# CVLAB-Unibo/MM2D3D

Measured on AMD Instinct MI355X. Metric: LiDAR scenes/sec fwd+bwd (NuScenes ~35k pts, 5cm voxel), higher is better.
Workload: dtype fp16 MFMA, fp32 accumulate, loss scale 65536 on the device (2D branch: IEEE fp16 maps and packed weights - the reference's precision: 16 = fp16 autocast + GradScaler) + f32 (3D sparse branch, fp32 as in the reference: f32 MFMA on narrow layers, fp32-faithful 3-term split-bf16 products with fp32 accu; 1 GPU; BASELINE.json configs[1]: NuScenes-shaped (32x1090 sweep, 34,880 pts/scene), 5 cm voxels, 480x302 RGB + sparse depth; full two-domain training step (train.py:186-292): 2D+3D fwd on source and target, 2 CE + 4 KL, backward, AdamW x2 + OneCycle; distinct_batches_rotated=4, parallelism=dp1

## Files before the change

include/mm2d3d.h:

```cpp
#ifndef MM2D3D_H
#define MM2D3D_H

#include <stddef.h>
#include <stdint.h>

#ifdef __cplusplus
extern "C" {
#endif

typedef void* mm_stream_t;

#define MM_OK 0
#define MM_ERR_ARG (-1)
#define MM_ERR_HIP (-2)
#define MM_ERR_WORKSPACE (-3)
#define MM_ERR_UNSUPPORTED (-4)

const char* mm_last_error(void);

typedef void* mm_handle_t;
size_t mm_handle_sync_bytes(void);
size_t mm_handle_fault_bytes(void);
int mm_create(int device_id, void* sync_dev, size_t sync_bytes, void* fault_host, size_t fault_bytes, mm_handle_t* out);
int mm_destroy(mm_handle_t h);
// ... 7 lines not shown
int mm_fault_poll(mm_handle_t h);


int64_t mm_hash_capacity(int64_t n_items);
size_t mm_dedupe_ws_bytes(int64_t n_bound);

int mm_voxel_dedupe(const void* coords, int coords_is_i64, int64_t n_bound, const int32_t* n_dev, int shift,
                    uint64_t* tkeys, int32_t* tvals, int64_t cap, int32_t* item2vox, int32_t* vox_coords,
                    int32_t* csr_off, int32_t* csr_items, int32_t* n_active_dev, int32_t* err_dev, int no_spin, void* ws,
                    size_t ws_bytes, mm_stream_t stream);

int mm_batch_lower_bound(const int32_t* vox_coords, const int32_t* n_dev, int32_t split, int32_t* out, mm_stream_t stream);
int mm_subm_neighbors(const int32_t* vox_coords, int64_t n, int32_t spatial_size, const uint64_t* tkeys,
                      const int32_t* tvals, int64_t cap, int32_t* nbr, mm_stream_t stream);

int mm_down_neighbors(const int32_t* vox_coords_fine, int64_t n_fine, const int32_t* fine2coarse, int64_t n_coarse,
                      int32_t* nbr, mm_stream_t stream);

size_t mm_rulebook_ws_bytes(int64_t n_out, int K);
int mm_rulebook_compact(const int32_t* nbr, int K, int64_t n_out, int32_t* rin, int32_t* rout, int32_t* offsets,
                        int32_t* csr_off, int32_t* csr_pos, int no_spin, void* ws, size_t ws_bytes, mm_stream_t stream);
int mm_rulebook_csr(const int32_t* nbr, int K, int64_t n_out, int32_t* csr_off, int32_t* csr_pos, int no_spin, void* ws,
                    size_t ws_bytes, mm_stream_t stream);

size_t mm_voxelize_ws_bytes(int64_t n_total, int B);
int mm_voxelize_batch(const float* points, const int32_t* scene_off_dev, const int32_t* scene_off_host, int B, const float* rot,
                      const double* u, int transl, float scale, int full_scale, int64_t* locs, int32_t* keep, int32_t* counts,
                      float* min_value, double* offset, void* ws, size_t ws_bytes, mm_stream_t stream);
size_t mm_voxelize_ws_bytes_f64(int64_t n_total, int B);
int mm_voxelize_batch_f64(const double* points, const int32_t* scene_off_dev, const int32_t* scene_off_host, int B, const float* rot,
                          const double* u, int transl, double scale, int full_scale, int64_t* locs, int32_t* keep, int32_t* counts,
                          double* min_value, double* offset, void* ws, size_t ws_bytes, mm_stream_t stream);
int mm_project_batch(const float* points_img, const float* depth_vals, const int64_t* labels, const int32_t* scene_off_dev,
                     const int32_t* scene_off_host, int B, int H, int W, const uint8_t* flip, int64_t* img_indices, float* depth,
                     double* seg2d, int32_t* winner, int32_t* err, mm_stream_t stream);
int mm_collect_points(const int32_t* keep, const int32_t* n_keep_dev, int64_t n_bound, const int64_t* locs, const int64_t* img_indices,
                      const int64_t* labels, const float* image, int C, int H, int W, const float* points, int64_t* img_indices_out,
                      int64_t* labels_out, float* feats_out, float* points_out, mm_stream_t stream);
int mm_collect_points_f64(const int32_t* keep, const int32_t* n_keep_dev, int64_t n_bound, const int64_t* locs, const int64_t* img_indices,
                          const int64_t* labels, const float* image, int C, int H, int W, const double* points, int64_t* img_indices_out,
                          int64_t* labels_out, float* feats_out, double* points_out, mm_stream_t stream);
int mm_collect_points_dev(const int32_t* keep, const int32_t* counts_dev, int B, int64_t n_total, const int64_t* locs,
                          const int64_t* img_indices, const int64_t* labels, const float* image, int C, int H, int W, const float* points,
                          int64_t* img_indices_out, int64_t* labels_out, float* feats_out, float* points_out,
                          const void* const* extra_in, void* const* extra_out, int n_extra, int extra_bytes, mm_stream_t stream);
int mm_collect_points_f64_dev(const int32_t* keep, const int32_t* counts_dev, int B, int64_t n_total, const int64_t* locs,
// ... 394 lines not shown
```

mm2d3d_amd/_lib.py:

```python
from __future__ import annotations

import contextlib
import ctypes as C
import os
import subprocess

import torch

_HERE = os.path.dirname(os.path.abspath(__file__))
LIB_PATH = os.environ.get("MM_LIB_PATH") or os.path.join(_HERE, "libmm2d3d_hip.so")
CSRC = os.path.join(_HERE, "csrc")

_lib = None

vp, i32, i64, sz, f32, f64 = C.c_void_p, C.c_int32, C.c_int64, C.c_size_t, C.c_float, C.c_double

_PROTOS = {
    "mm_last_error": (C.c_char_p, []),
    "mm_handle_sync_bytes": (sz, []),
    "mm_handle_fault_bytes": (sz, []),
    "mm_create": (i32, [i32, vp, sz, vp, sz, C.POINTER(vp)]),
    "mm_destroy": (i32, [vp]),
    "mm_set_option": (i32, [vp, i32, i32]),
    "mm_get_option": (i32, [vp, i32]),
    "mm_fault_poll": (i32, [vp]),
    "mm_hash_capacity": (i64, [i64]),
    "mm_dedupe_ws_bytes": (sz, [i64]),
    "mm_voxel_dedupe": (i32, [vp, i32, i64, vp, i32, vp, vp, i64, vp, vp, vp, vp, vp, vp, i32, vp, sz, vp]),
    "mm_batch_lower_bound": (i32, [vp, vp, i32, vp, vp]),
    "mm_subm_neighbors": (i32, [vp, i64, i32, vp, vp, i64, vp, vp]),
    "mm_down_neighbors": (i32, [vp, i64, vp, i64, vp, vp]),
    "mm_rulebook_ws_bytes": (sz, [i64, i32]),
    "mm_rulebook_compact": (i32, [vp, i32, i64, vp, vp, vp, vp, vp, i32, vp, sz, vp]),
    "mm_rulebook_csr": (i32, [vp, i32, i64, vp, vp, i32, vp, sz, vp]),
    "mm_spconv_ws_bytes": (sz, [i64, i32, i32, i32]),
    "mm_spconv_apply": (i32, [vp, i32, i32, vp, i32, i32, i64, vp, vp, vp, vp, i32, vp, vp, i32, vp, i64, i32, i32, i32, i32, vp, sz, vp]),
    "mm_spconv_apply_packed": (i32, [vp, i32, i32, vp, i32, i32, i64, vp, vp, vp, vp, i32, vp, vp, i32, vp, i64, i32, i32, i32, vp, i32, vp, sz, vp]),
    "mm_spconv_dw_ws_bytes": (sz, [vp, i32, i32, i32]),
    "mm_spconv_dw": (i32, [vp, i32, i32, vp, i32, i32, vp, vp, vp, i32, vp, i32, i32, vp, sz, vp]),
    "mm_voxelize_ws_bytes": (sz, [i64, i32]),
    "mm_voxelize_batch": (i32, [vp, vp, vp, i32, vp, vp, i32, f32, i32, vp, vp, vp, vp, vp, vp, sz, vp]),
    "mm_project_batch": (i32, [vp, vp, vp, vp, vp, i32, i32, i32, vp, vp, vp, vp, vp, vp, vp]),
    "mm_voxelize_ws_bytes_f64": (sz, [i64, i32]),
    "mm_voxelize_batch_f64": (i32, [vp, vp, vp, i32, vp, vp, i32, f64, i32, vp, vp, vp, vp, vp, vp, sz, vp]),
    "mm_collect_points": (i32, [vp, vp, i64, vp, vp, vp, vp, i32, i32, i32, vp, vp, vp, vp, vp, vp]),
    "mm_collect_points_f64": (i32, [vp, vp, i64, vp, vp, vp, vp, i32, i32, i32, vp, vp, vp, vp, vp, vp]),
    "mm_collect_points_dev": (i32, [vp, vp, i32, i64, vp, vp, vp, vp, i32, i32, i32, vp, vp, vp, vp, vp, vp, vp, i32, i32, vp]),
    "mm_collect_points_f64_dev": (i32, [vp, vp, i32, i64, vp, vp, vp, vp, i32, i32, i32, vp, vp, vp, vp, vp, vp, vp, i32, i32, vp]),
    "mm_image_prepare": (i32, [vp, i64, vp, vp, i32, i32, i32, vp, i64, vp, vp, vp, i64, vp, vp, vp, vp]),
    "mm_jpeg_ws_bytes": (sz, [i32, i64, i64, i64, i64, i64]),
    "mm_jpeg_decode": (i32, [vp, i64, vp, vp, i32, vp, i64, vp, i64, vp, i64, vp, vp, sz, vp]),
    "mm_up_neighbors": (i32, [vp, i64, vp, vp, vp]),
    "mm_os_table_ws_bytes": (sz, [i64, i32]),
    "mm_os_table_build": (i32, [vp, i32, i64, i32, i32, vp, vp, vp, vp, sz, vp]),
    "mm_spconv_os_pack_bytes": (sz, [i32, i32, i32]),
    "mm_spconv_os_pack_blocks": (i64, [i32, i32, i32]),
    "mm_spconv_os_pack_desc_fields": (i32, []),
# ... 118 lines not shown
    "mm_copy_rows_bf16": (i32, [vp, i64, vp, i64, i64, i32, vp]),
    "mm_concat_bf16": (i32, [vp, vp, i32, vp, i64, i32, vp]),
    "mm_maxpool3x3s2_fwd": (i32, [vp, i32, i32, i32, i32, i32, vp, vp, vp]),
    "mm_maxpool3x3s2_bwd": (i32, [vp, i32, vp, i32, vp, i32, i32, i32, i32, vp, vp]),
    "mm_head_ws_bytes": (sz, [i32, i32, i32, i32, i32, i32, i32]),
    "mm_head_fwd": (i32, [vp, i32, i32, i32, i32, i32, i32, i32, vp, vp, i32, vp, vp, sz, vp]),
    "mm_head_bwd": (i32, [vp, i32, i32, i32, i32, i32, i32, i32, vp, i32, vp, vp, vp, vp, sz, vp]),
}


class Bn2dFwdArgs(C.Structure):
    _fields_ = [("x", C.c_void_p), ("ld_x", C.c_int), ("res", C.c_void_p), ("ld_r", C.c_int), ("weight", C.c_void_p), ("bias", C.c_void_p),
                ("running_mean", C.c_void_p), ("running_var", C.c_void_p), ("num_batches_tracked", C.c_void_p), ("y", C.c_void_p),
                ("ld_y", C.c_int), ("save_mean", C.c_void_p), ("save_invstd", C.c_void_p)]


class Bn2dBwdArgs(C.Structure):
    _fields_ = [("x", C.c_void_p), ("ld_x", C.c_int), ("dy", C.c_void_p), ("ld_dy", C.c_int), ("dy2", C.c_void_p), ("ld_dy2", C.c_int),
                ("yout", C.c_void_p), ("ld_y", C.c_int), ("weight", C.c_void_p), ("bias", C.c_void_p), ("save_mean", C.c_void_p),
                ("save_invstd", C.c_void_p), ("dx", C.c_void_p), ("ld_dx", C.c_int), ("dres", C.c_void_p), ("ld_dr", C.c_int),
                ("dweight", C.c_void_p), ("dbias", C.c_void_p)]


class HipLibraryMissing(RuntimeError):
    pass


H16_2D = {
    "mm_conv2d_gemm": "mm_conv2d_gemm_f16",
    "mm_conv2d_dgrad_s2": "mm_conv2d_dgrad_s2_f16",
    "mm_conv2d_3x3s1": "mm_conv2d_3x3s1_f16",
    "mm_conv2d_3x3s1_pair": "mm_conv2d_3x3s1_pair_f16",
    "mm_conv2d_gemm_stat_rows": "mm_conv2d_gemm_stat_rows_f16",
    "mm_conv2d_3x3s1_stat_rows": "mm_conv2d_3x3s1_stat_rows_f16",
    "mm_bn2d_fwd_train_pre": "mm_bn2d_fwd_train_pre_f16",
    "mm_bn2d_single_launch": "mm_bn2d_single_launch_f16",
    "mm_bn2d_fwd_train_pair": "mm_bn2d_fwd_train_pair_f16",
    "mm_bn2d_fwd_train_pre_pool": "mm_bn2d_fwd_train_pre_pool_f16",
    "mm_bn2d_bwd_pool": "mm_bn2d_bwd_pool_f16",
    "mm_bn2d_bwd_pair": "mm_bn2d_bwd_pair_f16",
    "mm_conv2d_wgrad_ws_bytes": "mm_conv2d_wgrad_ws_bytes_f16",
    "mm_conv2d_wgrad": "mm_conv2d_wgrad_f16",
    "mm_conv2d_wgrad3x3_pair": "mm_conv2d_wgrad3x3_pair_f16",
    "mm_conv2d_wgrad_slabs": "mm_conv2d_wgrad_slabs_f16",
    "mm_conv2d_wgrad3x3_pair_slabs": "mm_conv2d_wgrad3x3_pair_slabs_f16",
    "mm_conv2d_wgrad_reduce_desc_bytes": "mm_conv2d_wgrad_reduce_desc_bytes_f16",
# ... 225 lines not shown
```

mm2d3d_amd/csrc/meta.hip:

```cpp
#include "common.h"

namespace {

constexpr unsigned long long EMPTY_KEY = 0xFFFFFFFFFFFFFFFFull;
constexpr int T = 256;

__device__ inline unsigned long long pack_key(int x, int y, int z, int b) {
  return ((unsigned long long)(unsigned)b << 48) | ((unsigned long long)(unsigned)x << 32) |
         ((unsigned long long)(unsigned)y << 16) | (unsigned long long)(unsigned)z;
}

__device__ inline unsigned long long mix64(unsigned long long k) {
  k ^= k >> 33;
  k *= 0xff51afd7ed558ccdull;
  k ^= k >> 33;
  k *= 0xc4ceb9fe1a85ec53ull;
  k ^= k >> 33;
  return k;
}

__device__ inline int hash_find(const unsigned long long* __restrict__ tkeys, const int32_t* __restrict__ tvals,
                                long long mask, unsigned long long key) {
  long long slot = (long long)(mix64(key) & (unsigned long long)mask);
  for (long long probe = 0; probe <= mask; probe++) {
// ... 186 lines not shown
  int64_t o = (int64_t)blockIdx.x * T + threadIdx.x;
  if (o >= n_out) return;
  int e = csr_off[o];
  for (int k = 0; k < K; k++)
    if (nbr[(int64_t)k * n_out + o] >= 0) csr_pos[e++] = pos[(int64_t)k * n_out + o];
}

__global__ void k_fill_i32(int32_t* p, int64_t n, int32_t v) {
  int64_t i = (int64_t)blockIdx.x * blockDim.x + threadIdx.x;
  if (i < n) p[i] = v;
}

inline unsigned nblk(int64_t n) { return (unsigned)mm_cdiv(n > 0 ? n : 1, T); }

__global__ void k_batch_lower_bound(const int32_t* __restrict__ coords, const int32_t* __restrict__ n_dev, int32_t split,
                                    int32_t* __restrict__ out) {
  int lo = 0, hi = *n_dev;
  while (lo < hi) {
    int mid = (lo + hi) >> 1;
    if (coords[(int64_t)mid * 4 + 3] < split) lo = mid + 1;
    else hi = mid;
  }
  *out = lo;
}
}

extern "C" {

int64_t mm_hash_capacity(int64_t n_items) {
  int64_t c = 1024;
  while (c < 2 * n_items) c <<= 1;
  return c;
}

size_t mm_dedupe_ws_bytes(int64_t n) { return 4 * mm_align((size_t)(n + 1) * 4) + mm_scan_ws_bytes(n + 1) + 1024; }

int mm_voxel_dedupe(const void* coords, int coords_is_i64, int64_t n_bound, const int32_t* n_dev, int shift,
                    uint64_t* tkeys, int32_t* tvals, int64_t cap, int32_t* item2vox, int32_t* vox_coords,
                    int32_t* csr_off, int32_t* csr_items, int32_t* n_active_dev, int32_t* err_dev, int no_spin, void* ws,
                    size_t ws_bytes, hipStream_t s) {
  MM_CHECK_ARG(n_bound >= 0 && cap >= 2 * n_bound && (cap & (cap - 1)) == 0, "dedupe: cap must be pow2 >= 2n (n=%lld cap=%lld)",
               (long long)n_bound, (long long)cap);
  MM_CHECK_ARG(shift >= 0 && shift < 16, "dedupe: bad shift %d", shift);
  MMArena ar(ws, ws_bytes);
  int32_t* slot_of = ar.take<int32_t>(n_bound + 1);
  int32_t* flag = ar.take<int32_t>(n_bound + 1);
// ... 82 lines not shown
  if (!pos || !cnt || !scan_ws) {
    mm_set_error("rulebook_compact: workspace too small (%zu < %zu)", ws_bytes, mm_rulebook_ws_bytes(n_out, K));
    return MM_ERR_WORKSPACE;
  }
  int rc = mm_exclusive_scan_nonneg_i32(nbr, pos, total, scan_ws, sws, s, no_spin);
  if (rc) return rc;
  if (rin) hipLaunchKernelGGL(k_emit_rules, dim3(nblk(n_out), K), dim3(T), 0, s, nbr, pos, n_out, K, rin, rout, offsets, pos + total);
  if (csr_off) {
    hipLaunchKernelGGL(k_row_counts, dim3(nblk(n_out)), dim3(T), 0, s, nbr, n_out, K, cnt);
    rc = mm_exclusive_scan_i32(cnt, csr_off, n_out, csr_off + n_out, scan_ws, sws, s, no_spin);
    if (rc) return rc;
    hipLaunchKernelGGL(k_row_fill, dim3(nblk(n_out)), dim3(T), 0, s, nbr, pos, n_out, K, csr_off, csr_pos);
  }
  MM_LAUNCH_CHECK();
  return MM_OK;
}

int mm_rulebook_csr(const int32_t* nbr, int K, int64_t n_out, int32_t* csr_off, int32_t* csr_pos, int no_spin, void* ws, size_t ws_bytes,
                    hipStream_t s) {
  MM_CHECK_ARG(csr_off && csr_pos, "rulebook_csr: null output");
  return mm_rulebook_compact(nbr, K, n_out, nullptr, nullptr, nullptr, csr_off, csr_pos, no_spin, ws, ws_bytes, s);
}

int mm_batch_lower_bound(const int32_t* vox_coords, const int32_t* n_dev, int32_t split, int32_t* out, hipStream_t s) {
  MM_CHECK_ARG(vox_coords && n_dev && out, "batch_lower_bound: null pointer");
  hipLaunchKernelGGL(k_batch_lower_bound, dim3(1), dim3(1), 0, s, vox_coords, n_dev, split, out);
  MM_LAUNCH_CHECK();
  return MM_OK;
}

}
```

mm2d3d_amd/csrc/scan.hip:

```cpp
#include <stdarg.h>

#include <rocprim/device/device_scan.hpp>
#include <rocprim/iterator/counting_iterator.hpp>
#include <rocprim/iterator/transform_iterator.hpp>

#include "common.h"

static thread_local char g_err[512] = "";
void mm_set_error(const char* fmt, ...) {
  va_list ap;
  va_start(ap, fmt);
  vsnprintf(g_err, sizeof(g_err), fmt, ap);
  va_end(ap);
}
extern "C" const char* mm_last_error() { return g_err; }

namespace {
constexpr int SCAN_T = 256;
constexpr int SCAN_PER = 8;
constexpr int SCAN_BLK = SCAN_T * SCAN_PER;

__device__ inline int wave_incl_scan(int v) {
  const int lane = threadIdx.x & 63;
#pragma unroll
// ... 15 lines not shown
  for (int i = 0; i < SCAN_T / 64; i++) {
    int x = wsum[i];
    if (i < w) base += x;
    total += x;
  }
  __syncthreads();
  *tot = total;
  return base + inc - v;
}

template <bool FLAG>
__global__ __launch_bounds__(SCAN_T) void k_block_sums(const int32_t* __restrict__ in, int32_t* __restrict__ sums,
                                                        int64_t n) {
  int64_t base = (int64_t)blockIdx.x * SCAN_BLK + threadIdx.x * SCAN_PER;
  int v = 0;
#pragma unroll
  for (int i = 0; i < SCAN_PER; i++)
    if (base + i < n) v += FLAG ? (in[base + i] >= 0 ? 1 : 0) : in[base + i];
  int tot;
  block_excl_scan(v, &tot);
  if (threadIdx.x == 0) sums[blockIdx.x] = tot;
}

__global__ __launch_bounds__(SCAN_T) void k_scan_sums(int32_t* __restrict__ sums, int64_t nb,
                                                       int32_t* __restrict__ total_out) {
  int carry = 0;
  for (int64_t b0 = 0; b0 < nb; b0 += SCAN_T) {
    int64_t i = b0 + threadIdx.x;
    int v = i < nb ? sums[i] : 0;
    int tot;
    int ex = block_excl_scan(v, &tot);
    if (i < nb) sums[i] = carry + ex;
    carry += tot;
  }
  if (threadIdx.x == 0 && total_out) *total_out = carry;
}

template <bool FLAG>
__global__ __launch_bounds__(SCAN_T) void k_rescan(const int32_t* __restrict__ in, int32_t* __restrict__ out,
                                                    const int32_t* __restrict__ sums, int64_t n) {
  int64_t base = (int64_t)blockIdx.x * SCAN_BLK + threadIdx.x * SCAN_PER;
  int x[SCAN_PER];
  int v = 0;
#pragma unroll
  for (int i = 0; i < SCAN_PER; i++) {
    x[i] = (base + i < n) ? (FLAG ? (in[base + i] >= 0 ? 1 : 0) : in[base + i]) : 0;
    v += x[i];
  }
  int tot;
  int ex = block_excl_scan(v, &tot) + sums[blockIdx.x];
#pragma unroll
  for (int i = 0; i < SCAN_PER; i++) {
    if (base + i < n) out[base + i] = ex;
    ex += x[i];
  }
// ... 75 lines not shown
```

mm2d3d_amd/scn/metadata.py:

```python
from __future__ import annotations

import contextlib
import os

import weakref

import numpy as np
import torch

from .. import _lib, domains
from .._lib import check, ptr, stream

I32 = torch.int32
NO_SPIN = [0]


@contextlib.contextmanager
def no_spin():
    prev, NO_SPIN[0] = NO_SPIN[0], 1
    try:
        yield
    finally:
        NO_SPIN[0] = prev

# ... 161 lines not shown
    def pending_tensors(self):
        if self._pending_rulebooks is not None:
            for _lv, subm, down in self._pending_rulebooks[1]:
                for rb in (subm, down):
                    if rb is not None:
                        yield from self._rulebook_tensors(rb)

    def build_levels(self, coords_i64: torch.Tensor):
        self.begin_levels(coords_i64)
        return self.finish_levels()

    def ensure(self):
        if self._pending_levels is not None:
            self.finish_levels()
        if self._pending_rulebooks is not None:
            self.finish_rulebooks()
        return self.levels[0]

    def begin_levels(self, coords_i64: torch.Tensor):
        L = _lib.lib()
        dev = self.device
        n_pts = self.n_points = coords_i64.shape[0]
        nlev = max(1, min(self.prebuild_levels, max(1, int(np.log2(max(self.spatial_size, 2))))))
        counts = torch.zeros(2 * nlev + 1, dtype=I32, device=dev)
        err = counts[nlev : nlev + 1]
        split = self.split = domains.current()
        cap = int(L.mm_hash_capacity(n_pts))
        ws = _lib.workspace.get(int(L.mm_dedupe_ws_bytes(n_pts)), dev)
        S = self.spatial_size
        prev = None
        for l in range(nlev):
            lv = Level(S)
            lv.cap = cap
            lv.tkeys = torch.empty(cap, dtype=torch.int64, device=dev)
            lv.tvals = torch.empty(cap, dtype=I32, device=dev)
            lv.item2vox = torch.empty(max(n_pts, 1), dtype=I32, device=dev)
            lv.coords = torch.empty((max(n_pts, 1), 4), dtype=I32, device=dev)
            lv.csr_off = torch.empty(n_pts + 1, dtype=I32, device=dev)
            lv.csr_items = torch.empty(max(n_pts, 1), dtype=I32, device=dev)
            if l == 0:
                src, is64, ndev, shift = coords_i64, 1, None, 0
            else:
                src, is64, ndev, shift = prev.coords, 0, ptr(counts[l - 1 : l]), 1
            check(
                L.mm_voxel_dedupe(ptr(src), is64, n_pts, ndev, shift, ptr(lv.tkeys), ptr(lv.tvals), cap,
                                  ptr(lv.item2vox), ptr(lv.coords), ptr(lv.csr_off), ptr(lv.csr_items),
                                  ptr(counts[l : l + 1]), ptr(err), NO_SPIN[0], ptr(ws), ws.numel(), stream()),
                "voxel_dedupe",
            )
            if split is not None:
                check(L.mm_batch_lower_bound(ptr(lv.coords), ptr(counts[l : l + 1]), split, ptr(counts[nlev + 1 + l : nlev + 2 + l]),
                                             stream()), "batch_lower_bound")
            if prev is not None:
                prev.coarse, lv.fine = lv, prev
            self.levels.append(lv)
            prev = lv
            S = max(S // 2, 1)
        self._pending_levels = (_Readback(counts), nlev, n_pts, split)

    def finish_levels(self):
        rb_, nlev, n_pts, split = self._pending_levels
        self._pending_levels = None
        host = rb_.wait()
        if host[nlev] != 0:
            raise ValueError("InputLayer: coordinates must satisfy 0 <= x,y,z,batch < 65536")
        n_items = n_pts
        for l, lv in enumerate(self.levels):
            lv.n = int(host[l])
            lv.seg_rows = int(host[nlev + 1 + l]) if split is not None else None
            lv.n_items = n_items
            lv.coords = lv.coords[: lv.n]
            lv.item2vox = lv.item2vox[:n_items]
            lv.csr_off = lv.csr_off[: lv.n + 1]
            lv.csr_items = lv.csr_items[:n_items]
            n_items = lv.n
# ... 11 lines not shown
        lv.coords = torch.empty((max(n, 1), 4), dtype=I32, device=dev)
        lv.csr_off = torch.empty(n + 1, dtype=I32, device=dev)
        lv.csr_items = torch.empty(max(n, 1), dtype=I32, device=dev)
        cnt = torch.zeros(3, dtype=I32, device=dev)
        ws = _lib.workspace.get(int(L.mm_dedupe_ws_bytes(n)), dev)
        check(
            L.mm_voxel_dedupe(ptr(fine.coords), 0, n, None, 1, ptr(lv.tkeys), ptr(lv.tvals), lv.cap, ptr(lv.item2vox),
                              ptr(lv.coords), ptr(lv.csr_off), ptr(lv.csr_items), ptr(cnt[0:1]), ptr(cnt[1:2]), NO_SPIN[0], ptr(ws),
                              ws.numel(), stream()),
            "voxel_dedupe",
        )
        if fine.seg_rows is not None:
            check(L.mm_batch_lower_bound(ptr(lv.coords), ptr(cnt[0:1]), self.split, ptr(cnt[2:3]), stream()), "batch_lower_bound")
        hc = cnt.cpu().numpy()
        lv.n = int(hc[0])
        lv.seg_rows = int(hc[2]) if fine.seg_rows is not None else None
        lv.n_items = n
        lv.coords = lv.coords[: lv.n]
        lv.csr_off = lv.csr_off[: lv.n + 1]
        fine.coarse, lv.fine = lv, fine
        self.levels.append(lv)
        return lv

    def _launch_rulebook(self, K, n_out, nbr, offsets_dev, with_csr=True):
        L = _lib.lib()
        dev = self.device
        rb = Rulebook(K)
        cap = max(K * n_out, 1)
        rb.rin = torch.empty(cap, dtype=I32, device=dev)
        rb.rout = torch.empty(cap, dtype=I32, device=dev)
        if with_csr:
            rb.csr_pos = torch.empty(cap, dtype=I32, device=dev)
            rb.csr_off = torch.empty(n_out + 1, dtype=I32, device=dev)
        else:
            rb.csr_pos = rb.csr_off = None
            rb.nbr = nbr
        rb.offsets_dev = offsets_dev
        rb.n_out = n_out
        ws = _lib.workspace.get(int(L.mm_rulebook_ws_bytes(n_out, K)), dev)
        check(
            L.mm_rulebook_compact(ptr(nbr), K, n_out, ptr(rb.rin), ptr(rb.rout), ptr(offsets_dev), ptr(rb.csr_off),
                                  ptr(rb.csr_pos), NO_SPIN[0], ptr(ws), ws.numel(), stream()),
            "rulebook_compact",
        )
        return rb

    def _os_table(self, nbr, K, n):
        if n == 0 or (n < OS_MIN_ROWS and not self.act16):
            return None
        L = _lib.lib()
        dev = self.device
        t = OsTable()
        t.K, t.n_dst, t.tile_rows = K, n, os_tile_rows(n)
        t.n_tiles = -(-n // t.tile_rows)
        npad = t.n_tiles * t.tile_rows
        t.dst = torch.empty(npad, dtype=I32, device=dev)
        t.nbrp = torch.empty(K * npad, dtype=I32, device=dev)
        t.tmask = torch.empty(t.n_tiles, dtype=I32, device=dev)
        ws = _lib.workspace.get(int(L.mm_os_table_ws_bytes(n, K)), dev)
        check(L.mm_os_table_build(ptr(nbr), K, n, t.tile_rows, NO_SPIN[0], ptr(t.dst), ptr(t.nbrp), ptr(t.tmask), ptr(ws), ws.numel(),
                                  stream()), "os_table_build")
        return t

    def build_rulebooks(self, levels=None):
        self.begin_rulebooks(levels)
        self.finish_rulebooks()

    def begin_rulebooks(self, levels=None):
        if self._pending_levels is not None:
            self.finish_levels()
        if self._pending_rulebooks is not None:
            self.finish_rulebooks()
        L = _lib.lib()
        dev = self.device
        levels = [lv for lv in (levels or self.levels) if lv.subm is None]
        if not levels:
            return
        offs = torch.zeros((len(levels), 28 + 9), dtype=I32, device=dev)
        pending = []
        for j, lv in enumerate(levels):
            nbr = torch.empty(max(27 * lv.n, 1), dtype=I32, device=dev)
            check(L.mm_subm_neighbors(ptr(lv.coords), lv.n, lv.spatial_size, ptr(lv.tkeys), ptr(lv.tvals), lv.cap,
                                      ptr(nbr), stream()), "subm_neighbors")
            subm_os = self._os_table(nbr, 27, lv.n)
            subm = self._launch_rulebook(27, lv.n, nbr, offs[j, :28], with_csr=subm_os is None)
            subm.os = subm_os
            down = None
            if lv.coarse is not None and lv.down is None:
                c = lv.coarse
                nbr8 = torch.empty(max(8 * c.n, 1), dtype=I32, device=dev)
                check(L.mm_down_neighbors(ptr(lv.coords), lv.n, ptr(c.item2vox), c.n, ptr(nbr8), stream()),
                      "down_neighbors")
                down_os = self._os_table(nbr8, 8, c.n)
                down = self._launch_rulebook(8, c.n, nbr8, offs[j, 28:37], with_csr=down_os is None)
                down.os = down_os
                if OS_BUILD_UP or self.act16:
                    nbr_up = torch.empty(max(8 * lv.n, 1), dtype=I32, device=dev)
                    check(L.mm_up_neighbors(ptr(lv.coords), lv.n, ptr(c.item2vox), ptr(nbr_up), stream()), "up_neighbors")
                    down.os_up = self._os_table(nbr_up, 8, lv.n)
            pending.append((lv, subm, down))
        self._pending_rulebooks = (_Readback(offs), pending)

    def finish_rulebooks(self):
        if self._pending_rulebooks is None:
            return
        rb_, pending = self._pending_rulebooks
        self._pending_rulebooks = None
        host = rb_.wait()
        for j, (lv, subm, down) in enumerate(pending):
            for rb, row in ((subm, host[j, :28]), (down, host[j, 28:37])):
                if rb is None:
                    continue
                rb.offsets_host = np.ascontiguousarray(row[: rb.K + 1], dtype=np.int32)
                rb.n_rules = int(rb.offsets_host[rb.K])
                rb.rin = rb.rin[: max(rb.n_rules, 1)]
                rb.rout = rb.rout[: max(rb.n_rules, 1)]
                if rb.csr_pos is not None:
                    rb.csr_pos = rb.csr_pos[: max(rb.n_rules, 1)]
            lv.subm = subm
            if down is not None:
                lv.down = down

    def subm_rulebook(self, lv: Level) -> Rulebook:
# ... 20 lines not shown
```

Measured before the change: 486.3 scenes/s.

## Batch multi-level voxel dedupe and rulebook construction into single launches

Replaces the per-level voxel dedupe loop (one dedupe plus batch lower-bound call per level, each chaining off the previous level) with one multi-level dedupe that hashes all pyramid levels in a single insert pass. The per-level scans, assign, fill and sort kernels now run with a level grid dimension. Neighbor generation and rulebook compaction for all levels are also batched into descriptor-driven kernels over shared buffers. The goal is fewer kernel launches and less host-side Python/ctypes overhead per scene. In exchange the code adds new kernels, larger combined workspaces and descriptor-lookup logic.

```diff
diff --git a/include/mm2d3d.h b/include/mm2d3d.h
--- a/include/mm2d3d.h
+++ b/include/mm2d3d.h
@@ -53,6 +53,23 @@
                         int32_t* csr_off, int32_t* csr_pos, int no_spin, void* ws, size_t ws_bytes, mm_stream_t stream);
 int mm_rulebook_csr(const int32_t* nbr, int K, int64_t n_out, int32_t* csr_off, int32_t* csr_pos, int no_spin, void* ws,
                     size_t ws_bytes, mm_stream_t stream);
+
+size_t mm_dedupe_levels_ws_bytes(int64_t n_pts, int nlev);
+int mm_voxel_dedupe_levels(const int64_t* coords, int64_t n_pts, int nlev, uint64_t* tkeys, int32_t* tvals, int64_t cap,
+                           int32_t* item2vox, int32_t* vox_coords, int32_t* csr_off, int32_t* csr_items, int32_t split,
+                           int32_t* counts, int no_spin, void* ws, size_t ws_bytes, mm_stream_t stream);
+#define MM_META_BATCH 32
+typedef struct mm_nbr_desc {
+  const int32_t* vox_coords; const uint64_t* tkeys; const int32_t* tvals; const int32_t* fine2coarse; int32_t* nbr;
+  int64_t n, n_coarse, cap; int32_t spatial_size, K;
+} mm_nbr_desc;
+int mm_neighbors_batch(const mm_nbr_desc* d, int nd, mm_stream_t stream);
+typedef struct mm_rulebook_desc {
+  int64_t start, n_out, row0, pos0; int32_t K, offs;
+} mm_rulebook_desc;
+size_t mm_rulebook_batch_ws_bytes(int64_t nbr_words, int64_t csr_rows);
+int mm_rulebook_compact_batch(const int32_t* nbr, const mm_rulebook_desc* d, int nd, int32_t* rin, int32_t* rout, int32_t* offsets,
+                              int32_t* csr_off, int32_t* csr_pos, int no_spin, void* ws, size_t ws_bytes, mm_stream_t stream);
 
 size_t mm_voxelize_ws_bytes(int64_t n_total, int B);
 int mm_voxelize_batch(const float* points, const int32_t* scene_off_dev, const int32_t* scene_off_host, int B, const float* rot,
diff --git a/mm2d3d_amd/_lib.py b/mm2d3d_amd/_lib.py
--- a/mm2d3d_amd/_lib.py
+++ b/mm2d3d_amd/_lib.py
@@ -33,6 +33,11 @@
     "mm_rulebook_ws_bytes": (sz, [i64, i32]),
     "mm_rulebook_compact": (i32, [vp, i32, i64, vp, vp, vp, vp, vp, i32, vp, sz, vp]),
     "mm_rulebook_csr": (i32, [vp, i32, i64, vp, vp, i32, vp, sz, vp]),
+    "mm_dedupe_levels_ws_bytes": (sz, [i64, i32]),
+    "mm_voxel_dedupe_levels": (i32, [vp, i64, i32, vp, vp, i64, vp, vp, vp, vp, i32, vp, i32, vp, sz, vp]),
+    "mm_neighbors_batch": (i32, [vp, i32, vp]),
+    "mm_rulebook_batch_ws_bytes": (sz, [i64, i64]),
+    "mm_rulebook_compact_batch": (i32, [vp, vp, i32, vp, vp, vp, vp, vp, i32, vp, sz, vp]),
     "mm_spconv_ws_bytes": (sz, [i64, i32, i32, i32]),
     "mm_spconv_apply": (i32, [vp, i32, i32, vp, i32, i32, i64, vp, vp, vp, vp, i32, vp, vp, i32, vp, i64, i32, i32, i32, i32, vp, sz, vp]),
     "mm_spconv_apply_packed": (i32, [vp, i32, i32, vp, i32, i32, i64, vp, vp, vp, vp, i32, vp, vp, i32, vp, i64, i32, i32, i32, vp, i32, vp, sz, vp]),
@@ -197,6 +202,15 @@
                 ("dweight", C.c_void_p), ("dbias", C.c_void_p)]
 
 
+class NbrDesc(C.Structure):
+    _fields_ = [("vox_coords", C.c_void_p), ("tkeys", C.c_void_p), ("tvals", C.c_void_p), ("fine2coarse", C.c_void_p), ("nbr", C.c_void_p),
+                ("n", C.c_int64), ("n_coarse", C.c_int64), ("cap", C.c_int64), ("spatial_size", C.c_int32), ("K", C.c_int32)]
+
+
+class RulebookDesc(C.Structure):
+    _fields_ = [("start", C.c_int64), ("n_out", C.c_int64), ("row0", C.c_int64), ("pos0", C.c_int64), ("K", C.c_int32), ("offs", C.c_int32)]
+
+
 class HipLibraryMissing(RuntimeError):
     pass
 
diff --git a/mm2d3d_amd/csrc/meta.hip b/mm2d3d_amd/csrc/meta.hip
--- a/mm2d3d_amd/csrc/meta.hip
+++ b/mm2d3d_amd/csrc/meta.hip
@@ -232,6 +232,271 @@
     else hi = mid;
   }
   *out = lo;
+}
+
+constexpr int MAX_LEVELS = 16;
+
+__global__ __launch_bounds__(T) void k_meta_init(unsigned long long* __restrict__ tkeys, int32_t* __restrict__ tvals, int64_t ntab,
+                                                  int32_t* __restrict__ cnt, int64_t ncnt, int32_t* __restrict__ counts, int ncounts) {
+  int64_t i = (int64_t)blockIdx.x * T + threadIdx.x;
+  if (i < ntab) {
+    tkeys[i] = ~0ull;
+    tvals[i] = 0x7F7F7F7F;
+  }
+  if (i < ncnt) cnt[i] = 0;
+  if (i < ncounts) counts[i] = 0;
+}
+
+__global__ __launch_bounds__(T) void k_meta_insert(const int64_t* __restrict__ coords, int64_t N, int L,
+                                                    unsigned long long* __restrict__ tkeys, int32_t* __restrict__ tvals, int64_t cap,
+                                                    int32_t* __restrict__ slot_of, int32_t* __restrict__ err) {
+  int64_t p = (int64_t)blockIdx.x * T + threadIdx.x;
+  if (p >= N) return;
+  long long x = coords[p * 4 + 0], y = coords[p * 4 + 1], z = coords[p * 4 + 2], b = coords[p * 4 + 3];
+  const bool bad = x < 0 || y < 0 || z < 0 || b < 0 || x > 65535 || y > 65535 || z > 65535 || b > 65535;
+  if (bad) atomicExch(err, 1);
+  const long long mask = cap - 1;
+  bool go = !bad;
+  for (int l = 0; l < L; l++) {
+    int32_t found = -1;
+    if (go) {
+      unsigned long long key = pack_key((int)(x >> l), (int)(y >> l), (int)(z >> l), (int)b);
+      unsigned long long* tk = tkeys + (int64_t)l * cap;
+      long long slot = (long long)(mix64(key) & (unsigned long long)mask);
+      for (long long probe = 0; probe <= mask; probe++) {
+        unsigned long long prev = atomicCAS(&tk[slot], EMPTY_KEY, key);
+        if (prev == EMPTY_KEY || prev == key) {
+          go = atomicMin(&tvals[(int64_t)l * cap + slot], (int32_t)p) > (int32_t)p;
+          found = (int32_t)slot;
+          break;
+        }
+        slot = (slot + 1) & mask;
+      }
+      if (found < 0) {
+        atomicExch(err, 2);
+        go = false;
+      }
+    }
+    slot_of[(int64_t)l * N + p] = found;
+  }
+}
+
+__global__ __launch_bounds__(T) void k_meta_flag_first(const int32_t* __restrict__ slot_of, const int32_t* __restrict__ tvals,
+                                                        int64_t N, int64_t cap, int32_t* __restrict__ flag) {
+  int64_t p = (int64_t)blockIdx.x * T + threadIdx.x;
+  const int l = blockIdx.y;
+  if (p >= N) return;
+  int s = slot_of[l * N + p];
+  flag[l * N + p] = (s >= 0 && tvals[l * cap + s] == (int32_t)p) ? 1 : 0;
+}
+
+__global__ __launch_bounds__(T) void k_meta_assign(const int64_t* __restrict__ coords, int64_t N, int64_t N1, int64_t cap,
+                                                    const int32_t* __restrict__ slot_of, const int32_t* __restrict__ tvals,
+                                                    const int32_t* __restrict__ rank, int32_t* __restrict__ flag,
+                                                    int32_t* __restrict__ item2vox, int32_t* __restrict__ vox_coords,
+                                                    int32_t* __restrict__ cnt, int32_t* __restrict__ counts) {
+  int64_t p = (int64_t)blockIdx.x * T + threadIdx.x;
+  const int l = blockIdx.y;
+  if (p >= N) return;
+  const int base = rank[l * N];
+  if (p == 0) counts[l] = rank[(l + 1) * N] - base;
+  flag[l * N + p] = 0;
+  int s = slot_of[l * N + p];
+  if (s < 0) {
+    if (l == 0) item2vox[p] = -1;
+    return;
+  }
+  int first = tvals[l * cap + s];
+  int v = rank[l * N + first] - base;
+  int64_t item = p;
+  bool is_item = true;
+  if (l > 0) {
+    const int r = rank[(l - 1) * N + p];
+    is_item = rank[(l - 1) * N + p + 1] != r;
+    item = r - rank[(l - 1) * N];
+  }
+  if (is_item) {
+    item2vox[l * N1 + item] = v;
+    atomicAdd(&cnt[l * N + v], 1);
+  }
+  if (first == (int32_t)p) {
+    int32_t* vc = vox_coords + (l * N1 + v) * 4;
+    vc[0] = (int32_t)(coords[p * 4 + 0] >> l);
+    vc[1] = (int32_t)(coords[p * 4 + 1] >> l);
+    vc[2] = (int32_t)(coords[p * 4 + 2] >> l);
+    vc[3] = (int32_t)coords[p * 4 + 3];
+  }
+}
+
+__global__ __launch_bounds__(T) void k_meta_fill(int64_t N, int64_t N1, int64_t cap, const int32_t* __restrict__ slot_of,
+                                                  const int32_t* __restrict__ rank, const int32_t* __restrict__ G,
+                                                  const int32_t* __restrict__ item2vox, int32_t* __restrict__ cursor,
+                                                  int32_t* __restrict__ tvals, int32_t* __restrict__ csr_off,
+                                                  int32_t* __restrict__ csr_items) {
+  int64_t p = (int64_t)blockIdx.x * T + threadIdx.x;
+  const int l = blockIdx.y;
+  if (p > N) return;
+  const int gbase = G[l * N];
+  csr_off[l * (N + 1) + p] = G[l * N + p] - gbase;
+  if (p == N) return;
+  const int r = rank[l * N + p];
+  if (rank[l * N + p + 1] != r) tvals[l * cap + slot_of[l * N + p]] = r - rank[l * N];
+  int64_t item = p;
+  if (l > 0) {
+    const int rf = rank[(l - 1) * N + p];
+    if (rank[(l - 1) * N + p + 1] == rf) return;
+    item = rf - rank[(l - 1) * N];
+  }
+  int v = item2vox[l * N1 + item];
+  if (v < 0) return;
+  int j = atomicAdd(&cursor[l * N + v], 1);
+  csr_items[l * N1 + (G[l * N + v] - gbase) + j] = (int32_t)item;
+}
+
+__global__ __launch_bounds__(T) void k_meta_sort_lists(int64_t N, int64_t N1, int L, const int32_t* __restrict__ csr_off,
+                                                        int32_t* __restrict__ csr_items, const int32_t* __restrict__ vox_coords,
+                                                        int32_t split, int32_t* __restrict__ counts) {
+  int64_t v = (int64_t)blockIdx.x * T + threadIdx.x;
+  const int l = blockIdx.y;
+  const int n = counts[l];
+  if (v == 0 && split >= 0) {
+    const int32_t* vc = vox_coords + l * N1 * 4;
+    int lo = 0, hi = n;
+    while (lo < hi) {
+      int mid = (lo + hi) >> 1;
+      if (vc[(int64_t)mid * 4 + 3] < split) lo = mid + 1;
+      else hi = mid;
+    }
+    counts[L + 1 + l] = lo;
+  }
+  if (v >= n) return;
+  const int32_t* off = csr_off + l * (N + 1);
+  int32_t* items = csr_items + l * N1;
+  int a = off[v], b = off[v + 1];
+  for (int i = a + 1; i < b; i++) {
+    int x = items[i];
+    int j = i - 1;
+    while (j >= a && items[j] > x) {
+      items[j + 1] = items[j];
+      j--;
+    }
+    items[j + 1] = x;
+  }
+}
+
+constexpr int MAX_BATCH = 32;
+struct NbrDesc {
+  const int32_t* vc; const unsigned long long* tkeys; const int32_t* tvals; const int32_t* f2c; int32_t* nbr;
+  int64_t n, n_coarse, cap; int32_t spatial, K;
+};
+struct NbrBatch {
+  NbrDesc d[MAX_BATCH];
+  unsigned first[MAX_BATCH + 1];
+};
+struct RbDesc {
+  int64_t start, n_out, row0, pos0; int32_t K, offs;
+};
+struct RbBatch {
+  RbDesc d[MAX_BATCH];
+  unsigned first[MAX_BATCH + 1];
+};
+
+__device__ inline int find_task(const unsigned* first, unsigned blk) {
+  int j = 0;
+  while (first[j + 1] <= blk) j++;
+  return j;
+}
+
+__global__ __launch_bounds__(T) void k_meta_nbr_fill(const NbrBatch tb) {
+  const int j = find_task(tb.first, blockIdx.x);
+  const NbrDesc& d = tb.d[j];
+  int64_t i = (int64_t)(blockIdx.x - tb.first[j]) * T + threadIdx.x;
+  if (d.K == 27) {
+    if (i < 13 * d.n) d.nbr[14 * d.n + i] = -1;
+  } else if (i < 8 * d.n_coarse) {
+    d.nbr[i] = -1;
+  }
+}
+
+__global__ __launch_bounds__(T) void k_meta_subm_nbr(const NbrBatch tb) {
+  const int j = find_task(tb.first, blockIdx.x);
+  const NbrDesc& d = tb.d[j];
+  const int32_t* __restrict__ vc = d.vc;
+  int32_t* __restrict__ nbr = d.nbr;
+  const int64_t n = d.n;
+  int64_t o = (int64_t)(blockIdx.x - tb.first[j]) * T + threadIdx.x;
+  int k = blockIdx.y;
+  if (o >= n) return;
+  if (k == 13) {
+    nbr[(int64_t)13 * n + o] = (int)o;
+    return;
+  }
+  int x = vc[o * 4 + 0] + (k / 9 - 1), y = vc[o * 4 + 1] + ((k / 3) % 3 - 1), z = vc[o * 4 + 2] + (k % 3 - 1);
+  int b = vc[o * 4 + 3];
+  int r = -1;
+  const int spatial = d.spatial;
+  if (x >= 0 && y >= 0 && z >= 0 && x < spatial && y < spatial && z < spatial)
+    r = hash_find(d.tkeys, d.tvals, (long long)(d.cap - 1), pack_key(x, y, z, b));
+  nbr[(int64_t)k * n + o] = r;
+  if (r >= 0) nbr[(int64_t)(26 - k) * n + r] = (int)o;
+}
+
+__global__ __launch_bounds__(T) void k_meta_down_nbr(const NbrBatch tb) {
+  const int j = find_task(tb.first, blockIdx.x);
+  const NbrDesc& d = tb.d[j];
+  const int32_t* __restrict__ vc = d.vc;
+  int64_t i = (int64_t)(blockIdx.x - tb.first[j]) * T + threadIdx.x;
+  if (i >= d.n) return;
+  int k = ((vc[i * 4 + 0] & 1) * 2 + (vc[i * 4 + 1] & 1)) * 2 + (vc[i * 4 + 2] & 1);
+  d.nbr[(int64_t)k * d.n_coarse + d.f2c[i]] = (int32_t)i;
+}
+
+__global__ __launch_bounds__(T) void k_meta_emit_rules(const RbBatch tb, const int32_t* __restrict__ nbr, const int32_t* __restrict__ pos,
+                                                        int32_t* __restrict__ rin, int32_t* __restrict__ rout,
+                                                        int32_t* __restrict__ offsets) {
+  const int j = find_task(tb.first, blockIdx.x);
+  const RbDesc& d = tb.d[j];
+  const int64_t n = d.n_out;
+  const unsigned nb = (unsigned)((n + T - 1) / T), lb = blockIdx.x - tb.first[j];
+  const int k = (int)(lb / nb);
+  const int64_t o = (int64_t)(lb - k * nb) * T + threadIdx.x;
+  if (o >= n) return;
+  const int64_t e = k * n + o;
+  const int base = pos[d.start];
+  const int p = pos[d.start + e] - base;
+  if (o == 0) offsets[d.offs + k] = p;
+  if (e == 0) offsets[d.offs + d.K] = pos[d.start + d.K * n] - base;
+  int i = nbr[d.start + e];
+  if (i >= 0) {
+    rin[d.start + p] = i;
+    rout[d.start + p] = (int32_t)o;
+  }
+}
+
+__global__ __launch_bounds__(T) void k_meta_row_counts(const RbBatch tb, const int32_t* __restrict__ nbr, int32_t* __restrict__ cnt) {
+  const int j = find_task(tb.first, blockIdx.x);
+  const RbDesc& d = tb.d[j];
+  int64_t o = (int64_t)(blockIdx.x - tb.first[j]) * T + threadIdx.x;
+  if (o > d.n_out) return;
+  int c = 0;
+  if (o < d.n_out)
+    for (int k = 0; k < d.K; k++) c += nbr[d.start + k * d.n_out + o] >= 0;
+  cnt[d.row0 + o] = c;
+}
+
+__global__ __launch_bounds__(T) void k_meta_row_fill(const RbBatch tb, const int32_t* __restrict__ nbr, const int32_t* __restrict__ pos,
+                                                      const int32_t* __restrict__ G, int32_t* __restrict__ csr_off,
+                                                      int32_t* __restrict__ csr_pos) {
+  const int j = find_task(tb.first, blockIdx.x);
+  const RbDesc& d = tb.d[j];
+  int64_t o = (int64_t)(blockIdx.x - tb.first[j]) * T + threadIdx.x;
+  if (o > d.n_out) return;
+  int e = G[d.row0 + o] - G[d.row0];
+  csr_off[d.row0 + o] = e;
+  if (o == d.n_out) return;
+  const int base = pos[d.start];
+  for (int k = 0; k < d.K; k++)
+    if (nbr[d.start + k * d.n_out + o] >= 0) csr_pos[d.pos0 + e++] = pos[d.start + k * d.n_out + o] - base;
 }
 }
 
@@ -360,6 +625,140 @@
   return mm_rulebook_compact(nbr, K, n_out, nullptr, nullptr, nullptr, csr_off, csr_pos, no_spin, ws, ws_bytes, s);
 }
 
+size_t mm_dedupe_levels_ws_bytes(int64_t n_pts, int nlev) {
+  const int64_t m = (int64_t)nlev * n_pts + 1;
+  return 5 * mm_align((size_t)m * 4) + mm_scan_ws_bytes(m) + 1024;
+}
+
+int mm_voxel_dedupe_levels(const int64_t* coords, int64_t n_pts, int nlev, uint64_t* tkeys, int32_t* tvals, int64_t cap,
+                           int32_t* item2vox, int32_t* vox_coords, int32_t* csr_off, int32_t* csr_items, int32_t split,
+                           int32_t* counts, int no_spin, void* ws, size_t ws_bytes, hipStream_t s) {
+  const int64_t N = n_pts, N1 = N > 0 ? N : 1, M = (int64_t)nlev * N;
+  MM_CHECK_ARG(N >= 0 && nlev >= 1 && nlev <= MAX_LEVELS && cap >= 2 * N && (cap & (cap - 1)) == 0 && M < (1ll << 31),
+               "dedupe_levels: 1 <= nlev <= %d, cap must be pow2 >= 2n, nlev * n < 2^31 (n=%lld nlev=%d cap=%lld)", MAX_LEVELS,
+               (long long)N, nlev, (long long)cap);
+  MMArena ar(ws, ws_bytes);
+  int32_t* slot_of = ar.take<int32_t>(M + 1);
+  int32_t* flag = ar.take<int32_t>(M + 1);
+  int32_t* rank = ar.take<int32_t>(M + 1);
+  int32_t* cnt = ar.take<int32_t>(M + 1);
+  int32_t* G = ar.take<int32_t>(M + 1);
+  size_t sws = mm_scan_ws_bytes(M + 1);
+  char* scan_ws = ar.take<char>(sws);
+  if (!slot_of || !flag || !rank || !cnt || !G || !scan_ws) {
+    mm_set_error("dedupe_levels: workspace too small (%zu < %zu)", ws_bytes, mm_dedupe_levels_ws_bytes(N, nlev));
+    return MM_ERR_WORKSPACE;
+  }
+  {
+    const int64_t ntab = (int64_t)nlev * cap;
+    int64_t ni = ntab > M + 1 ? ntab : M + 1;
+    if (ni < 2 * nlev + 1) ni = 2 * nlev + 1;
+    hipLaunchKernelGGL(k_meta_init, dim3(nblk(ni)), dim3(T), 0, s, (unsigned long long*)tkeys, tvals, ntab, cnt, M + 1, counts,
+                       2 * nlev + 1);
+  }
+  if (N == 0) {
+    MM_HIP(hipMemsetAsync(csr_off, 0, (size_t)nlev * 4, s));
+    return MM_OK;
+  }
+  const unsigned g = nblk(N);
+  hipLaunchKernelGGL(k_meta_insert, dim3(g), dim3(T), 0, s, coords, N, nlev, (unsigned long long*)tkeys, tvals, cap, slot_of,
+                     counts + nlev);
+  hipLaunchKernelGGL(k_meta_flag_first, dim3(g, nlev), dim3(T), 0, s, slot_of, tvals, N, cap, flag);
+  int rc = mm_exclusive_scan_i32(flag, rank, M, rank + M, scan_ws, sws, s, no_spin);
+  if (rc) return rc;
+  hipLaunchKernelGGL(k_meta_assign, dim3(g, nlev), dim3(T), 0, s, coords, N, N1, cap, slot_of, tvals, rank, flag, item2vox, vox_coords,
+                     cnt, counts);
+  rc = mm_exclusive_scan_i32(cnt, G, M, G + M, scan_ws, sws, s, no_spin);
+  if (rc) return rc;
+  hipLaunchKernelGGL(k_meta_fill, dim3(nblk(N + 1), nlev), dim3(T), 0, s, N, N1, cap, slot_of, rank, G, item2vox, flag, tvals, csr_off,
+                     csr_items);
+  hipLaunchKernelGGL(k_meta_sort_lists, dim3(g, nlev), dim3(T), 0, s, N, N1, nlev, csr_off, csr_items, vox_coords, split, counts);
+  MM_LAUNCH_CHECK();
+  return MM_OK;
+}
+
+int mm_neighbors_batch(const NbrDesc* d, int nd, hipStream_t s) {
+  MM_CHECK_ARG(d && nd >= 0 && nd <= MAX_BATCH, "neighbors_batch: at most %d tables", MAX_BATCH);
+  NbrBatch fill, subm, down;
+  unsigned nf = 0, ns = 0, ndn = 0;
+  for (int j = 0; j < nd; j++) {
+    const NbrDesc& t = d[j];
+    MM_CHECK_ARG((t.K == 27 || t.K == 8) && t.n >= 0 && t.n_coarse >= 0 && (t.K == 8 || (t.cap & (t.cap - 1)) == 0),
+                 "neighbors_batch: bad table %d", j);
+    fill.d[j] = subm.d[j] = down.d[j] = t;
+    fill.first[j] = nf, subm.first[j] = ns, down.first[j] = ndn;
+    if (t.K == 27) {
+      nf += (unsigned)mm_cdiv(13 * t.n, T);
+      ns += (unsigned)mm_cdiv(t.n, T);
+    } else if (t.n_coarse > 0) {
+      nf += (unsigned)mm_cdiv(8 * t.n_coarse, T);
+      ndn += (unsigned)mm_cdiv(t.n, T);
+    }
+  }
+  for (int j = nd; j <= MAX_BATCH; j++) fill.first[j] = nf, subm.first[j] = ns, down.first[j] = ndn;
+  if (nf) hipLaunchKernelGGL(k_meta_nbr_fill, dim3(nf), dim3(T), 0, s, fill);
+  if (ns) hipLaunchKernelGGL(k_meta_subm_nbr, dim3(ns, 14), dim3(T), 0, s, subm);
+  if (ndn) hipLaunchKernelGGL(k_meta_down_nbr, dim3(ndn), dim3(T), 0, s, down);
+  MM_LAUNCH_CHECK();
+  return MM_OK;
+}
+
+size_t mm_rulebook_batch_ws_bytes(int64_t nbr_words, int64_t csr_rows) {
+  return mm_align((size_t)(nbr_words + 1) * 4) + 2 * mm_align((size_t)(csr_rows + 1) * 4) +
+         mm_scan_ws_bytes((nbr_words > csr_rows ? nbr_words : csr_rows) + 1) + 1024;
+}
+
+int mm_rulebook_compact_batch(const int32_t* nbr, const RbDesc* d, int nd, int32_t* rin, int32_t* rout, int32_t* offsets,
+                              int32_t* csr_off, int32_t* csr_pos, int no_spin, void* ws, size_t ws_bytes, hipStream_t s) {
+  MM_CHECK_ARG(d && nd >= 0 && nd <= MAX_BATCH, "rulebook_compact_batch: at most %d tables", MAX_BATCH);
+  RbBatch emit, rows;
+  int64_t total = 0, nrows = 0;
+  unsigned ne = 0, nr = 0;
+  int nc = 0;
+  for (int j = 0; j < nd; j++) {
+    const RbDesc& t = d[j];
+    MM_CHECK_ARG(t.K > 0 && t.K <= 64 && t.n_out >= 0 && t.start == total && (t.row0 < 0 || (t.row0 == nrows && csr_off && csr_pos)),
+                 "rulebook_compact_batch: table %d does not follow the one before", j);
+    if (t.n_out == 0) MM_HIP(hipMemsetAsync(offsets + t.offs, 0, (size_t)(t.K + 1) * 4, s));
+    emit.d[j] = t;
+    emit.first[j] = ne;
+    ne += (unsigned)(t.K * mm_cdiv(t.n_out, T));
+    total += t.K * t.n_out;
+    if (t.row0 >= 0) {
+      rows.d[nc] = t;
+      rows.first[nc++] = nr;
+      nr += (unsigned)mm_cdiv(t.n_out + 1, T);
+      nrows += t.n_out + 1;
+    }
+  }
+  MM_CHECK_ARG(total < (1ll << 31), "rulebook_compact_batch: %lld table words", (long long)total);
+  for (int j = nd; j <= MAX_BATCH; j++) emit.first[j] = ne;
+  for (int j = nc; j <= MAX_BATCH; j++) rows.first[j] = nr;
+  MMArena ar(ws, ws_bytes);
+  int32_t* pos = ar.take<int32_t>(total + 1);
+  int32_t* cnt = ar.take<int32_t>(nrows + 1);
+  int32_t* G = ar.take<int32_t>(nrows + 1);
+  size_t sws = mm_scan_ws_bytes((total > nrows ? total : nrows) + 1);
+  char* scan_ws = ar.take<char>(sws);
+  if (!pos || !cnt || !G || !scan_ws) {
+    mm_set_error("rulebook_compact_batch: workspace too small (%zu < %zu)", ws_bytes, mm_rulebook_batch_ws_bytes(total, nrows));
+    return MM_ERR_WORKSPACE;
+  }
+  if (total) {
+    int rc = mm_exclusive_scan_nonneg_i32(nbr, pos, total, scan_ws, sws, s, no_spin);
+    if (rc) return rc;
+    hipLaunchKernelGGL(k_meta_emit_rules, dim3(ne), dim3(T), 0, s, emit, nbr, pos, rin, rout, offsets);
+  }
+  if (nrows) {
+    hipLaunchKernelGGL(k_meta_row_counts, dim3(nr), dim3(T), 0, s, rows, nbr, cnt);
+    int rc = mm_exclusive_scan_i32(cnt, G, nrows, G + nrows, scan_ws, sws, s, no_spin);
+    if (rc) return rc;
+    hipLaunchKernelGGL(k_meta_row_fill, dim3(nr), dim3(T), 0, s, rows, nbr, pos, G, csr_off, csr_pos);
+  }
+  MM_LAUNCH_CHECK();
+  return MM_OK;
+}
+
 int mm_batch_lower_bound(const int32_t* vox_coords, const int32_t* n_dev, int32_t split, int32_t* out, hipStream_t s) {
   MM_CHECK_ARG(vox_coords && n_dev && out, "batch_lower_bound: null pointer");
   hipLaunchKernelGGL(k_batch_lower_bound, dim3(1), dim3(1), 0, s, vox_coords, n_dev, split, out);
diff --git a/mm2d3d_amd/csrc/scan.hip b/mm2d3d_amd/csrc/scan.hip
--- a/mm2d3d_amd/csrc/scan.hip
+++ b/mm2d3d_amd/csrc/scan.hip
@@ -61,15 +61,26 @@
   if (threadIdx.x == 0) sums[blockIdx.x] = tot;
 }
 
+constexpr int SUMS_PER = 16;
 __global__ __launch_bounds__(SCAN_T) void k_scan_sums(int32_t* __restrict__ sums, int64_t nb,
                                                        int32_t* __restrict__ total_out) {
   int carry = 0;
-  for (int64_t b0 = 0; b0 < nb; b0 += SCAN_T) {
-    int64_t i = b0 + threadIdx.x;
-    int v = i < nb ? sums[i] : 0;
+  for (int64_t b0 = 0; b0 < nb; b0 += SCAN_T * SUMS_PER) {
+    const int64_t i0 = b0 + (int64_t)threadIdx.x * SUMS_PER;
+    int x[SUMS_PER];
+    int v = 0;
+#pragma unroll
+    for (int j = 0; j < SUMS_PER; j++) {
+      x[j] = i0 + j < nb ? sums[i0 + j] : 0;
+      v += x[j];
+    }
     int tot;
-    int ex = block_excl_scan(v, &tot);
-    if (i < nb) sums[i] = carry + ex;
+    int ex = carry + block_excl_scan(v, &tot);
+#pragma unroll
+    for (int j = 0; j < SUMS_PER; j++) {
+      if (i0 + j < nb) sums[i0 + j] = ex;
+      ex += x[j];
+    }
     carry += tot;
   }
   if (threadIdx.x == 0 && total_out) *total_out = carry;
diff --git a/mm2d3d_amd/scn/metadata.py b/mm2d3d_amd/scn/metadata.py
--- a/mm2d3d_amd/scn/metadata.py
+++ b/mm2d3d_amd/scn/metadata.py
@@ -207,35 +207,28 @@
         dev = self.device
         n_pts = self.n_points = coords_i64.shape[0]
         nlev = max(1, min(self.prebuild_levels, max(1, int(np.log2(max(self.spatial_size, 2))))))
-        counts = torch.zeros(2 * nlev + 1, dtype=I32, device=dev)
-        err = counts[nlev : nlev + 1]
+        counts = torch.empty(2 * nlev + 1, dtype=I32, device=dev)
         split = self.split = domains.current()
         cap = int(L.mm_hash_capacity(n_pts))
-        ws = _lib.workspace.get(int(L.mm_dedupe_ws_bytes(n_pts)), dev)
+        ws = _lib.workspace.get(int(L.mm_dedupe_levels_ws_bytes(n_pts, nlev)), dev)
+        n1 = max(n_pts, 1)
+        tkeys = torch.empty((nlev, cap), dtype=torch.int64, device=dev)
+        tvals = torch.empty((nlev, cap), dtype=I32, device=dev)
+        item2vox = torch.empty((nlev, n1), dtype=I32, device=dev)
+        coords = torch.empty((nlev, n1, 4), dtype=I32, device=dev)
+        csr_off = torch.empty((nlev, n_pts + 1), dtype=I32, device=dev)
+        csr_items = torch.empty((nlev, n1), dtype=I32, device=dev)
+        check(
+            L.mm_voxel_dedupe_levels(ptr(coords_i64), n_pts, nlev, ptr(tkeys), ptr(tvals), cap, ptr(item2vox), ptr(coords), ptr(csr_off),
+                                     ptr(csr_items), -1 if split is None else split, ptr(counts), NO_SPIN[0], ptr(ws), ws.numel(), stream()),
+            "voxel_dedupe_levels",
+        )
         S = self.spatial_size
         prev = None
         for l in range(nlev):
             lv = Level(S)
             lv.cap = cap
-            lv.tkeys = torch.empty(cap, dtype=torch.int64, device=dev)
-            lv.tvals = torch.empty(cap, dtype=I32, device=dev)
-            lv.item2vox = torch.empty(max(n_pts, 1), dtype=I32, device=dev)
-            lv.coords = torch.empty((max(n_pts, 1), 4), dtype=I32, device=dev)
-            lv.csr_off = torch.empty(n_pts + 1, dtype=I32, device=dev)
-            lv.csr_items = torch.empty(max(n_pts, 1), dtype=I32, device=dev)
-            if l == 0:
-                src, is64, ndev, shift = coords_i64, 1, None, 0
-            else:
-                src, is64, ndev, shift = prev.coords, 0, ptr(counts[l - 1 : l]), 1
-            check(
-                L.mm_voxel_dedupe(ptr(src), is64, n_pts, ndev, shift, ptr(lv.tkeys), ptr(lv.tvals), cap,
-                                  ptr(lv.item2vox), ptr(lv.coords), ptr(lv.csr_off), ptr(lv.csr_items),
-                                  ptr(counts[l : l + 1]), ptr(err), NO_SPIN[0], ptr(ws), ws.numel(), stream()),
-                "voxel_dedupe",
-            )
-            if split is not None:
-                check(L.mm_batch_lower_bound(ptr(lv.coords), ptr(counts[l : l + 1]), split, ptr(counts[nlev + 1 + l : nlev + 2 + l]),
-                                             stream()), "batch_lower_bound")
+            lv.tkeys, lv.tvals, lv.item2vox, lv.coords, lv.csr_off, lv.csr_items = tkeys[l], tvals[l], item2vox[l], coords[l], csr_off[l], csr_items[l]
             if prev is not None:
                 prev.coarse, lv.fine = lv, prev
             self.levels.append(lv)
@@ -293,31 +286,11 @@
         self.levels.append(lv)
         return lv
 
-    def _launch_rulebook(self, K, n_out, nbr, offsets_dev, with_csr=True):
-        L = _lib.lib()
-        dev = self.device
-        rb = Rulebook(K)
-        cap = max(K * n_out, 1)
-        rb.rin = torch.empty(cap, dtype=I32, device=dev)
-        rb.rout = torch.empty(cap, dtype=I32, device=dev)
-        if with_csr:
-            rb.csr_pos = torch.empty(cap, dtype=I32, device=dev)
-            rb.csr_off = torch.empty(n_out + 1, dtype=I32, device=dev)
-        else:
-            rb.csr_pos = rb.csr_off = None
-            rb.nbr = nbr
-        rb.offsets_dev = offsets_dev
-        rb.n_out = n_out
-        ws = _lib.workspace.get(int(L.mm_rulebook_ws_bytes(n_out, K)), dev)
-        check(
-            L.mm_rulebook_compact(ptr(nbr), K, n_out, ptr(rb.rin), ptr(rb.rout), ptr(offsets_dev), ptr(rb.csr_off),
-                                  ptr(rb.csr_pos), NO_SPIN[0], ptr(ws), ws.numel(), stream()),
-            "rulebook_compact",
-        )
-        return rb
+    def _takes_os(self, n):
+        return n != 0 and (n >= OS_MIN_ROWS or self.act16)
 
     def _os_table(self, nbr, K, n):
-        if n == 0 or (n < OS_MIN_ROWS and not self.act16):
+        if not self._takes_os(n):
             return None
         L = _lib.lib()
         dev = self.device
@@ -348,28 +321,54 @@
         if not levels:
             return
         offs = torch.zeros((len(levels), 28 + 9), dtype=I32, device=dev)
-        pending = []
+        pending, tabs = [], []
+        total = rows = npos = 0
         for j, lv in enumerate(levels):
-            nbr = torch.empty(max(27 * lv.n, 1), dtype=I32, device=dev)
-            check(L.mm_subm_neighbors(ptr(lv.coords), lv.n, lv.spatial_size, ptr(lv.tkeys), ptr(lv.tvals), lv.cap,
-                                      ptr(nbr), stream()), "subm_neighbors")
-            subm_os = self._os_table(nbr, 27, lv.n)
-            subm = self._launch_rulebook(27, lv.n, nbr, offs[j, :28], with_csr=subm_os is None)
-            subm.os = subm_os
-            down = None
+            subm, down = Rulebook(27), None
+            subm.n_out = lv.n
             if lv.coarse is not None and lv.down is None:
-                c = lv.coarse
-                nbr8 = torch.empty(max(8 * c.n, 1), dtype=I32, device=dev)
-                check(L.mm_down_neighbors(ptr(lv.coords), lv.n, ptr(c.item2vox), c.n, ptr(nbr8), stream()),
-                      "down_neighbors")
-                down_os = self._os_table(nbr8, 8, c.n)
-                down = self._launch_rulebook(8, c.n, nbr8, offs[j, 28:37], with_csr=down_os is None)
-                down.os = down_os
-                if OS_BUILD_UP or self.act16:
-                    nbr_up = torch.empty(max(8 * lv.n, 1), dtype=I32, device=dev)
-                    check(L.mm_up_neighbors(ptr(lv.coords), lv.n, ptr(c.item2vox), ptr(nbr_up), stream()), "up_neighbors")
-                    down.os_up = self._os_table(nbr_up, 8, lv.n)
+                down = Rulebook(8)
+                down.n_out = lv.coarse.n
+            for rb, o in ((subm, 37 * j), (down, 37 * j + 28)):
+                if rb is None:
+                    continue
+                csr = not self._takes_os(rb.n_out)
+                tabs.append((rb, lv, total, rows if csr else -1, npos, o))
+                total += rb.K * rb.n_out
+                if csr:
+                    rows += rb.n_out + 1
+                    npos += rb.K * rb.n_out
             pending.append((lv, subm, down))
+        nbr, rin, rout = (torch.empty(max(total, 1), dtype=I32, device=dev) for _ in range(3))
+        csr_off = torch.empty(max(rows, 1), dtype=I32, device=dev)
+        csr_pos = torch.empty(max(npos, 1), dtype=I32, device=dev)
+        nd, rd = (_lib.NbrDesc * len(tabs))(), (_lib.RulebookDesc * len(tabs))()
+        for i, (rb, lv, start, row0, pos0, o) in enumerate(tabs):
+            w = rb.K * rb.n_out
+            rb.nbr, rb.rin, rb.rout = nbr[start : start + w], rin[start : start + w], rout[start : start + w]
+            rb.offsets_dev = offs.view(-1)[o : o + rb.K + 1]
+            if row0 >= 0:
+                rb.csr_off, rb.csr_pos = csr_off[row0 : row0 + rb.n_out + 1], csr_pos[pos0 : pos0 + w]
+            else:
+                rb.csr_off = rb.csr_pos = None
+            if rb.K == 27:
+                nd[i] = _lib.NbrDesc(ptr(lv.coords), ptr(lv.tkeys), ptr(lv.tvals), None, ptr(rb.nbr), lv.n, 0, lv.cap, lv.spatial_size, 27)
+            else:
+                nd[i] = _lib.NbrDesc(ptr(lv.coords), None, None, ptr(lv.coarse.item2vox), ptr(rb.nbr), lv.n, lv.coarse.n, 0, 0, 8)
+            rd[i] = _lib.RulebookDesc(start, rb.n_out, row0, pos0, rb.K, o)
+        check(L.mm_neighbors_batch(nd, len(tabs), stream()), "neighbors_batch")
+        for rb, lv, *_ in tabs:
+            rb.os = self._os_table(rb.nbr, rb.K, rb.n_out)
+            if rb.K == 8 and (OS_BUILD_UP or self.act16):
+                nbr_up = torch.empty(max(8 * lv.n, 1), dtype=I32, device=dev)
+                check(L.mm_up_neighbors(ptr(lv.coords), lv.n, ptr(lv.coarse.item2vox), ptr(nbr_up), stream()), "up_neighbors")
+                rb.os_up = self._os_table(nbr_up, 8, lv.n)
+        ws = _lib.workspace.get(int(L.mm_rulebook_batch_ws_bytes(total, rows)), dev)
+        check(L.mm_rulebook_compact_batch(ptr(nbr), rd, len(tabs), ptr(rin), ptr(rout), ptr(offs), ptr(csr_off), ptr(csr_pos), NO_SPIN[0],
+                                          ptr(ws), ws.numel(), stream()), "rulebook_compact_batch")
+        for rb, *_ in tabs:
+            if rb.csr_pos is not None:
+                rb.nbr = None
         self._pending_rulebooks = (_Readback(offs), pending)
 
     def finish_rulebooks(self):
```

Result: faster. 492.1 scenes/s, median of 6 (+1.2%).
